# cipherflow-fhe/lattisense

Hardware: AMD Instinct MI355X
Metric: ckks_hmult_relin_rescale_throughput (higher is better)
Workload: dtype u64

## Files before the change

### lattisense_amd/csrc/build_flags.h

```cpp
#pragma once

#if (defined(LSA_NTT_DIAG_NO_TWIDDLE_LOADS) || defined(LSA_NTT_DIAG_COPY_ONLY) || defined(LSA_NTT_DIAG_COMPUTE_ONLY) || defined(LSA_NTT_DIAG_TW8) || \
     defined(LSA_KS_DIAG_NO_MATH) || defined(LSA_KS_DIAG_NO_STORE) || defined(LSA_BC_DIAG_NO_MATH) || defined(LSA_BC_DIAG_NO_STORE)) && \
    !defined(LSA_DIAG_BUILD)
#error "wrong-result diagnostic switches need -DLSA_DIAG_BUILD (use lattisense_amd.build --variant: it adds the flag and renames the library)"
#endif

#define LSA_BF_STR2(x) #x
#define LSA_BF_STR(x) LSA_BF_STR2(x)

#define LSA_BUILD_FLAGS_TEXT_1 ""
#ifdef LSA_DIAG_BUILD
#define LSA_BF_DIAG " LSA_DIAG_BUILD"
#else
#define LSA_BF_DIAG ""
#endif
#ifdef LSA_NTT_DIAG_NO_TWIDDLE_LOADS
#define LSA_BF_A " LSA_NTT_DIAG_NO_TWIDDLE_LOADS"
#else
#define LSA_BF_A ""
#endif
#ifdef LSA_NTT_DIAG_COPY_ONLY
#define LSA_BF_B " LSA_NTT_DIAG_COPY_ONLY"
#else
// ... 54 lines not shown
#else
#define LSA_BF_M ""
#endif
#ifdef LSA_BC_CARRY_COMPARES
#define LSA_BF_N " LSA_BC_CARRY_COMPARES"
#else
#define LSA_BF_N ""
#endif
#if defined(LSA_NTT_THREADS) && LSA_NTT_THREADS != 256
#define LSA_BF_O " LSA_NTT_THREADS=" LSA_BF_STR(LSA_NTT_THREADS)
#else
#define LSA_BF_O ""
#endif
#if defined(LSA_NTT_MAX_RHO) && LSA_NTT_MAX_RHO != 4
#define LSA_BF_P " LSA_NTT_MAX_RHO=" LSA_BF_STR(LSA_NTT_MAX_RHO)
#else
#define LSA_BF_P ""
#endif
#if defined(LSA_NTT_WAVES) && LSA_NTT_WAVES != 4
#define LSA_BF_Q " LSA_NTT_WAVES=" LSA_BF_STR(LSA_NTT_WAVES)
#else
#define LSA_BF_Q ""
#endif
#if defined(LSA_NTT_WAVES_FUSED) && LSA_NTT_WAVES_FUSED != 3
#define LSA_BF_R " LSA_NTT_WAVES_FUSED=" LSA_BF_STR(LSA_NTT_WAVES_FUSED)
#else
#define LSA_BF_R ""
#endif
#if defined(LSA_NTT_TAU) && LSA_NTT_TAU != 12
#define LSA_BF_S " LSA_NTT_TAU=" LSA_BF_STR(LSA_NTT_TAU)
#else
#define LSA_BF_S ""
#endif
#if defined(LSA_NTT_STORE_CHUNK) && LSA_NTT_STORE_CHUNK != 4
#define LSA_BF_T " LSA_NTT_STORE_CHUNK=" LSA_BF_STR(LSA_NTT_STORE_CHUNK)
#else
#define LSA_BF_T ""
#endif
#if defined(LSA_NTT_HEAD_ROUNDS) && LSA_NTT_HEAD_ROUNDS != 2
#define LSA_BF_U " LSA_NTT_HEAD_ROUNDS=" LSA_BF_STR(LSA_NTT_HEAD_ROUNDS)
#else
#define LSA_BF_U ""
#endif
#ifdef LSA_R16_BARRIERS
#define LSA_BF_X " LSA_R16_BARRIERS"
#else
#define LSA_BF_X ""
#endif
#if defined(LSA_R16_WAVES) && LSA_R16_WAVES != 4
#define LSA_BF_Y " LSA_R16_WAVES=" LSA_BF_STR(LSA_R16_WAVES)
#else
#define LSA_BF_Y ""
#endif
#ifdef LSA_NTT_NO_LAZY
#define LSA_BF_Z " LSA_NTT_NO_LAZY"
#else
#define LSA_BF_Z ""
#endif
#ifdef LSA_SHOUP_SINGLE_ASM
#define LSA_BF_AA " LSA_SHOUP_SINGLE_ASM"
#else
#define LSA_BF_AA ""
#endif
#ifdef LSA_AB_DPP_LO
#define LSA_BF_AB " LSA_AB_DPP_LO"
#else
#define LSA_BF_AB ""
#endif
#if defined(LSA_KSMAC_WAVES) && LSA_KSMAC_WAVES != 2
#define LSA_BF_AC " LSA_KSMAC_WAVES=" LSA_BF_STR(LSA_KSMAC_WAVES)
#else
#define LSA_BF_AC ""
#endif
#if defined(LSA_KSMAC_WAVES_FP) && LSA_KSMAC_WAVES_FP != 2
#define LSA_BF_AE " LSA_KSMAC_WAVES_FP=" LSA_BF_STR(LSA_KSMAC_WAVES_FP)
#else
#define LSA_BF_AE ""
#endif
#if defined(LSA_KSMAC_CHUNK) && LSA_KSMAC_CHUNK != 4
#define LSA_BF_AF " LSA_KSMAC_CHUNK=" LSA_BF_STR(LSA_KSMAC_CHUNK)
#else
#define LSA_BF_AF ""
#endif
#ifdef LSA_NTT_DIAG_TW8
#define LSA_BF_AD " LSA_NTT_DIAG_TW8"
#else
#define LSA_BF_AD ""
#endif
#ifdef LSA_LIFT_ROW_OUTER
#define LSA_BF_AG " LSA_LIFT_ROW_OUTER"
#else
#define LSA_BF_AG ""
#endif
#ifdef LSA_VARIANT_NAME
#define LSA_BF_V " variant=" LSA_BF_STR(LSA_VARIANT_NAME)
#else
#define LSA_BF_V ""
#endif
#ifdef LSA_AB_SWITCH
#define LSA_BF_W " LSA_AB_SWITCH=" LSA_BF_STR(LSA_AB_SWITCH)
#else
#define LSA_BF_W ""
#endif

#define LSA_BUILD_FLAGS_TEXT                                                                                              \
    LSA_BF_DIAG LSA_BF_A LSA_BF_B LSA_BF_C LSA_BF_D LSA_BF_E LSA_BF_F LSA_BF_G LSA_BF_H LSA_BF_I LSA_BF_J LSA_BF_K LSA_BF_L \
        LSA_BF_M LSA_BF_N LSA_BF_O LSA_BF_P LSA_BF_Q LSA_BF_R LSA_BF_S LSA_BF_T LSA_BF_U LSA_BF_V LSA_BF_W LSA_BF_X LSA_BF_Y LSA_BF_Z LSA_BF_AA LSA_BF_AB LSA_BF_AC LSA_BF_AD LSA_BF_AE LSA_BF_AF LSA_BF_AG
```

### lattisense_amd/csrc/kernels.hip

```cpp
#include <atomic>
#include <cstdlib>

#include "build_flags.h"
#include "lsa_internal.h"
#include "ntt_r16.h"
#include "plain_ops.h"
#include "poly_lincomb.h"
#include "tensor_sum.h"

namespace lsa {

const char* kernels_build_flags() { return LSA_BUILD_FLAGS_TEXT; }

static constexpr int TPB = 256;

#ifndef LSA_NTT_WAVES
#define LSA_NTT_WAVES 4
#endif

#if defined(LSA_NTT_DIAG_STAMPS)
#define LSA_STAMP(k)                                                                               \
    do {                                                                                           \
        if (a.diag && threadIdx.x == 0 && blockIdx.x < 8192) a.diag[blockIdx.x * 8 + (k)] = __builtin_amdgcn_s_memtime(); \
    } while (0)
// ... 136 lines not shown
}
static bool ntt_launch_r16(const NttPassArgs& a, int npass, bool fused, long long nblocks, hipStream_t s) {
    if (!sw::ntt_r16() || !ntt_r16_shape_ok(a, npass)) return false;
    const int fz = ntt_pass_fz(a, fused);
    void (*k)(NttPassArgs) = nullptr;
    if (a.lambda) {
        if (fz == 1 && a.fz_pro == 4 && sw::r16_pro()) k = a.mu == 8 ? &k_ntt_r16<0, 32, 8> : &k_ntt_r16<0, 32, 7>;
        else if (fz == 1 && a.fz_pro != 4 && a.mu == 8 && sw::r16_pro()) k = &k_ntt_r16<0, 1, 8>;
        else if (fz == 0) k = a.mu == 8 ? &k_ntt_r16<0, 0, 8> : &k_ntt_r16<0, 0, 7>;
    } else if (a.mu != 9 || sw::ntt_r8x3()) {
        switch (fz) {
            case 0: k = ntt_r16_second_pass<0>(a.mu); break;
            case 2: k = ntt_r16_second_pass<2>(a.mu); break;
            case 4: k = ntt_r16_second_pass<4>(a.mu); break;
            case 8: k = ntt_r16_second_pass<8>(a.mu); break;
            case 16: k = a.inverse ? ntt_r16_second_pass<16>(a.mu) : nullptr; break;
        }
    }
    if (!k) return false;
    hipLaunchKernelGGL(k, dim3((unsigned)nblocks), dim3(LSA_R16_THREADS), (size_t)LSA_R16_LDS_WORDS * sizeof(u64), s, a);
    LSA_HIP(hipGetLastError());
    return true;
}

#ifndef LSA_KSMAC_WAVES
#define LSA_KSMAC_WAVES 2
#endif
#ifndef LSA_KSMAC_WAVES_FP
#define LSA_KSMAC_WAVES_FP LSA_KSMAC_WAVES
#endif
template <int MU, bool FP, bool TAIL = false>
__global__ __launch_bounds__(LSA_R16_THREADS, FP ? LSA_KSMAC_WAVES_FP : LSA_KSMAC_WAVES) void k_ntt_r16_ksmac(KsFusedArgs g) {
    static_assert(!TAIL || (FP && MU <= 8), "the tail runs on the FP64 engine's eight- and seven-stage passes");
    extern __shared__ __attribute__((aligned(16))) u64 lds[];
    const int tid = threadIdx.x;
    const int T = g.L + g.np;
    long long bid = blockIdx.x;
    long long b;
    if (g.xcd_deal) {
        const long long slot = bid >> 3;
        b = slot % g.batch;
        bid = (slot / g.batch) * 8 + (bid & 7);
    } else {
        b = bid % g.batch;
        bid /= g.batch;
    }
    const int tl = g.tl_list[bid % g.n_tl], tile = (int)(bid / g.n_tl);
    NttPassArgs a;
    a.logn = g.logn;
    a.s_lo = g.logn - MU;
    a.mu = MU;
    a.lambda = 0;
    a.tau = 12;
    a.inverse = 0;
    a.apply_scale = 0;
    a.final_reduce = 1;
    a.fp_raw_in = g.fp_raw_in;
    a.fp_raw_out = 0;
    a.mods = g.mods;
    a.tw = g.tw;
    a.twd = g.twd;
    a.scale = nullptr;
    a.scaled = nullptr;
    a.src = g.ext;
    a.fz_pro = a.fz_epi = 0;
    a.fz_first = 0;
    NttBlockCtx bc;
    bc.tile = tile;
    bc.mod = tl < g.L ? tl : g.nq + (tl - g.L);
    bc.fp = FP;
    bc.b = (int)b;
    bc.row = 0;
    bc.tw_l = nullptr;
    bc.base_dst = 0;
    const R16Limb L = r16_limb(a, bc);
    const int kj = tl < g.L ? tl : g.klvl + 1 + (tl - g.L);
    const int own_d = tl < g.L ? tl / g.np : -1;
    int k, i;
    r16_lane<1, MU>(tid, k, i);
    const unsigned G1 = r16_G1<1, MU>(bc, k), G2 = (G1 << 4) + ((unsigned)i << (MU <= 8 ? 8 - MU : 0));
    u64 acc0[16], acc1[16];
#pragma unroll
    for (int e = 0; e < 16; e++) acc0[e] = acc1[e] = 0;
    for (int d = 0; d < g.beta; d++) {
        const bool own = d == own_d;
        if (!own) {
            bc.base_src = b * g.sext + ((long long)(d * T + tl) << g.logn);
            bc.row = d * T + tl;
            u64 v[16];
            r16_load_direct<1, false, 0, MU>(a, bc, tid, v);
            if constexpr (MU == 9) {
                r8x3_group<0>(v, a, bc, L, G1, i);
                r8x3_put<0>(k, i, lds, v);
                r16_sync<1>();
                r8x3_get<1>(k, i, lds, v);
                r8x3_group<1>(v, a, bc, L, G1, i);
                r8x3_put<1>(k, i, lds, v);
                r16_sync<1>();
                r8x3_get<2>(k, i, lds, v);
                r8x3_group<2>(v, a, bc, L, G1, i);
                r8x3_put<2>(k, i, lds, v);
            } else {
                r16_group<1, 0, MU>(v, a, bc, L, G1);
                r16_lds_put<1, 0, MU>(tid, lds, v);
                r16_sync<1>();
                r16_lds_get<1, 1, MU>(tid, lds, v);
                r16_group<1, 1, MU>(v, a, bc, L, G2);
                r16_lds_put<1, 1, MU>(tid, lds, v);
            }
            r16_sync<1>();
        }
        r16_mac_digit<MU, FP>(g, a, bc, L, tid, d, kj, own, b, tl, lds, acc0, acc1);
        r16_sync<1>();
    }
    if constexpr (TAIL) {
        a.src = g.tconv;
        int tt = tid, ttl = tl;
        long long tb = b;
        asm volatile("" : "+v"(tt), "+s"(ttl), "+s"(tb));
        int tk, ti;
        r16_lane<1, MU>(tt, tk, ti);
        const unsigned T1 = r16_G1<1, MU>(bc, tk), T2 = (T1 << 4) + ((unsigned)ti << (8 - MU));
        const double kd = g.tkd[ttl], k2d = g.tkd[g.L - 1 + ttl];
#pragma unroll 1
        for (int h = 0; h < 2; h++) {
            bc.row = h * g.L + ttl;
            bc.base_src = tb * g.stconv + ((long long)bc.row << g.logn);
            u64 v[16];
            r16_load_direct<1, false, 0, MU>(a, bc, tt, v);
            r16_group<1, 0, MU>(v, a, bc, L, T1);
            r16_lds_put<1, 0, MU>(tt, lds, v);
            r16_sync<1>();
            r16_lds_get<1, 1, MU>(tt, lds, v);
            r16_group<1, 1, MU>(v, a, bc, L, T2);
            r16_lds_put<1, 1, MU>(tt, lds, v);
            r16_sync<1>();
            r16_mac_tail<MU>(g, a, bc, L, tt, tb, ttl, h, kd, k2d, lds, acc0);
            r16_sync<1>();
#pragma unroll
            for (int e = 0; e < 16; e++) acc0[e] = acc1[e];
        }
        return;
    }
    r16_mac_store<MU, FP>(g, a, bc, L, tid, b, tl, acc0, acc1);
}

bool ks_fused_enabled(const Context& c) {
    if (!sw::ks_fused() || c.plan.npass != 2 || !c.fp_raw) return false;
    const NttPassShape& p = c.plan.pass[1];
    return p.tau == 12 && p.lambda == 0 && (p.mu == 7 || p.mu == 8 || p.mu == 9) && p.s_lo == c.logn - p.mu;
}

int ks_fused_engines(const Context& c) {
    return c.fp64_ntt ? sw::ks_fused_engines() : 0;
}

bool ks_fused_limb(const Context& c, int L, int tl) { return (ks_fused_engines(c) >> (c.fp_engine(c.qp_mod(L, tl)) ? 1 : 0)) & 1; }

bool launch_ntt_ksmac(Context& c, int level, const u64* cx, long long scx, u64* ext, long long sext, const Key& key, u64* acc,
                      long long sacc, int batch, hipStream_t s, const TensorFold* fold, KsFusedLimbs limbs, const KsTailOperands* tail) {
    if (batch <= 0) return true;
    if (!ks_fused_enabled(c) || (c.fp64_ntt && !key.fp)) return false;
    LSA_REQUIRE(key.level >= level, "key-switch key exported at a lower level than the ciphertext");
    LSA_REQUIRE((limbs == KS_FUSED_Q_TAIL) == (tail != nullptr), "fused key MAC: the tail launch and its operands go together");
    if (tail && (level < 1 || ks_fused_engines(c) != 2 || c.plan.pass[1].mu > 8)) return false;
    KsFusedArgs g{};
    if (tail) {
        g.tconv = tail->conv;
        g.stconv = tail->sconv;
        g.tout = tail->out;
        g.stout = tail->sout;
        g.tkd = reinterpret_cast<const double*>(c.tail_fp_vec(level));
    }
    g.ext = ext;
    g.cx = cx;
    g.key = key.data;
    g.keyd = key.fp;
    g.acc = acc;
    g.sext = sext;
    g.scx = scx;
    g.sacc = sacc;
    g.mods = c.d_mods;
    g.tw = c.d_psi;
    g.twd = c.d_psi_d;
    g.logn = c.logn;
    g.L = level + 1;
    g.np = c.np;
    g.nq = c.nq;
    g.beta = (g.L + c.np - 1) / c.np;
    g.klvl = key.level;
    g.kcomp = key.level + 1 + c.np;
    g.batch = batch;
    g.allow_fp64 = c.fp64_ntt;
    g.fp_raw_in = c.fp_raw;
    if (fold) {
        g.fa = fold->a;
        g.fb = fold->b;
        g.sfa = fold->sa;
        g.sfb = fold->sb;
        g.pfa = fold->pa;
        g.pfb = fold->pb;
        g.pf = c.pfold_vec(level);
    }
    const int T = g.L + c.np, mu = c.plan.pass[1].mu;
    LSA_REQUIRE(T <= 64, "fused key MAC: too many target limbs");
    const size_t lds_bytes = (size_t)LSA_R16_LDS_WORDS * sizeof(u64);
    for (int eng = 0; eng < 2; eng++) {
        g.n_tl = 0;
        int transforms = 0, q_targets = 0;
        for (int tl = 0; tl < T; tl++) {
            if (!ks_fused_limb(c, g.L, tl) || (int)c.fp_engine(c.qp_mod(g.L, tl)) != eng) continue;
            if (limbs == KS_FUSED_P && tl < g.L) continue;
            if (limbs == KS_FUSED_Q_TAIL && tl >= level) continue;
            g.tl_list[g.n_tl++] = (unsigned char)tl;
            transforms += g.beta - (tl < g.L ? 1 : 0);
            q_targets += tl < g.L;
        }
        if (!g.n_tl) continue;
        const long long nblocks = (long long)batch * g.n_tl * (1 << (c.logn - 12));
        LSA_REQUIRE(nblocks < (1LL << 31), "ntt: grid too large");
        g.xcd_deal = sw::ksmac_xcd() && ((g.n_tl << (c.logn - 12)) % 8 == 0) ? 1 : 0;
        if (tail) transforms += 2 * g.n_tl;
        const double ntt_bytes = 16.0 * c.n * transforms * batch / 2;
        const double fold_bytes = fold ? 3.0 * 8 * c.n * q_targets * batch : 0.0;
        ProfScope ps(c, PROF_NTT, ntt_bytes + fold_bytes + 8.0 * c.n * g.n_tl * (batch * ((double)g.beta + (tail ? 0.0 : 2.0)) + 2.0 * g.beta), s,
                     ntt_bytes);
        const dim3 grid((unsigned)nblocks), block(LSA_R16_THREADS);
        if (tail) {
            LSA_REQUIRE(eng == 1 && (mu == 8 || mu == 7), "fused key MAC: the tail runs on the FP64 engine's eight- and seven-stage passes");
            if (mu == 8) hipLaunchKernelGGL((k_ntt_r16_ksmac<8, true, true>), grid, block, lds_bytes, s, g);
            else hipLaunchKernelGGL((k_ntt_r16_ksmac<7, true, true>), grid, block, lds_bytes, s, g);
        } else if (mu == 9 && eng) hipLaunchKernelGGL((k_ntt_r16_ksmac<9, true>), grid, block, lds_bytes, s, g);
        else if (mu == 9) hipLaunchKernelGGL((k_ntt_r16_ksmac<9, false>), grid, block, lds_bytes, s, g);
        else if (mu == 8 && eng) hipLaunchKernelGGL((k_ntt_r16_ksmac<8, true>), grid, block, lds_bytes, s, g);
        else if (mu == 8) hipLaunchKernelGGL((k_ntt_r16_ksmac<8, false>), grid, block, lds_bytes, s, g);
        else if (eng) hipLaunchKernelGGL((k_ntt_r16_ksmac<7, true>), grid, block, lds_bytes, s, g);
        else hipLaunchKernelGGL((k_ntt_r16_ksmac<7, false>), grid, block, lds_bytes, s, g);
    }
    LSA_HIP(hipGetLastError());
    return true;
}

template <int FZ, int NT>
static void ntt_launch_variant(const NttPassArgs& a, long long nblocks, size_t lds_bytes, hipStream_t s) {
    if (lds_bytes > 65536) {
        static std::atomic<unsigned long long> raised{0};
        int dev = 0;
        LSA_HIP(hipGetDevice(&dev));
        const unsigned long long bit = 1ull << (dev & 63);
        if (!(raised.load(std::memory_order_acquire) & bit)) {
            LSA_HIP(hipFuncSetAttribute(reinterpret_cast<const void*>(&k_ntt_pass<FZ, NT>), hipFuncAttributeMaxDynamicSharedMemorySize, 160 * 1024));
            raised.fetch_or(bit, std::memory_order_release);
        }
    }
    hipLaunchKernelGGL((k_ntt_pass<FZ, NT>), dim3((unsigned)nblocks), dim3(NT), lds_bytes, s, a);
    LSA_HIP(hipGetLastError());
}

template <int NT>
static void ntt_launch_pass(const NttPassArgs& a, bool fused, long long nblocks, size_t lds_bytes, hipStream_t s) {
    LSA_REQUIRE((1 << a.tau) <= 2 * LSA_NTT_STAGE_PAIRS * NT, "ntt: tile larger than the staging registers");
    switch (ntt_pass_fz(a, fused)) {
        case 0: ntt_launch_variant<0, NT>(a, nblocks, lds_bytes, s); break;
        case 1: ntt_launch_variant<1, NT>(a, nblocks, lds_bytes, s); break;
        case 2: ntt_launch_variant<2, NT>(a, nblocks, lds_bytes, s); break;
        case 3: ntt_launch_variant<3, NT>(a, nblocks, lds_bytes, s); break;
        case 4: ntt_launch_variant<4, NT>(a, nblocks, lds_bytes, s); break;
        case 8: ntt_launch_variant<8, NT>(a, nblocks, lds_bytes, s); break;
        default:
            if constexpr (NT == LSA_NTT_THREADS) ntt_launch_variant<16, NT>(a, nblocks, lds_bytes, s);
            else LSA_REQUIRE(false, "ntt: the product prologue needs a tile of at most 4096 points");
    }
}

void launch_ntt(Context& c, const u64* src, u64* dst, int batch, long long batch_stride, int rows, const RowMap& rm,
                bool inverse, hipStream_t s) {
    launch_ntt(c, src, dst, batch, batch_stride, batch_stride, rows, rm, inverse, s);
}

void launch_ntt(Context& c, const u64* src, u64* dst, int batch, long long src_stride, long long dst_stride, int rows,
                const RowMap& rm, bool inverse, hipStream_t s, const NttFusion* fz, int passes) {
    if (batch <= 0 || rows <= 0) return;
    LSA_REQUIRE(rm.period >= 1 && rm.period <= LSA_MAX_PERIOD, "ntt: bad row-map period");
    NttPassArgs a{};
    a.batch = batch;
    a.rows = rows;
    a.mods = c.d_mods;
    a.scale = c.d_scale;
    a.diag = c.ntt_diag;
    a.scaled = c.d_scale_d;
    a.allow_fp64 = c.fp64_ntt;
    if (fz) {
        LSA_REQUIRE(!inverse || (fz->pro == 3 && !fz->epi), "inverse transforms take the product prologue only");
        LSA_REQUIRE(fz->pro != 3 || (inverse && !fz->epi && fz->a && fz->b && fz->limbs >= 1 && (passes & 1)),
                    "product prologue: an inverse transform from its first pass, two operands, no epilogue");
        LSA_REQUIRE(fz->pro != 4 || (!inverse && !fz->epi && fz->last && fz->limbs >= 1 && (passes & 1)),
                    "lift prologue: a forward transform from its first pass, one source row per polynomial, no epilogue");
        a.fz_epi = fz->epi;
        a.fz_pro = fz->pro;
        a.fz_limbs = fz->limbs;
        a.fz_base_polys = fz->base_polys;
        a.fz_ql_mod = fz->ql_mod;
        a.fz_a = fz->a;
        a.fz_a_stride = fz->a_stride;
        a.fz_a_rpp = fz->a_rpp;
        a.fz_base = fz->base;
        a.fz_base_stride = fz->base_stride;
        a.fz_base_rpp = fz->base_rpp;
        a.fz_k = fz->k;
        a.fz_out = fz->out;
        a.fz_out_stride = fz->out_stride;
        a.fz_out_rpp = fz->out_rpp;
        a.fz_last = fz->last;
        a.fz_last_stride = fz->last_stride;
        a.fz_last_rpp = fz->last_rpp;
        a.fz_k2 = fz->k2;
        a.fz_scatter = fz->scatter;
        LSA_REQUIRE(fz->epi != 2 || fz->k2, "merged tail needs its second factor");
        LSA_REQUIRE(!fz->scatter || fz->epi, "a scattered store needs an epilogue");
        LSA_REQUIRE(fz->epi != 3 || (!fz->pro && !fz->scatter && fz->a && fz->out), "pt_mul epilogue: plaintext and output, nothing else");
// ... 2089 lines not shown
```

### lattisense_amd/csrc/ntt_core.h

```cpp
#pragma once
#include "modarith.h"

#ifndef LSA_NTT_THREADS
#define LSA_NTT_THREADS 256
#endif
#define LSA_MAX_PERIOD 192
#if defined(LSA_EMULATE)
#include <cstdio>
#include <cstdlib>
#define LSA_EMU_CHECK(c) do { if (!(c)) { std::fprintf(stderr, "ntt replay: range invariant violated: %s (%s:%d)\n", #c, __FILE__, __LINE__); std::abort(); } } while (0)
#else
#define LSA_EMU_CHECK(c) do { } while (0)
#endif
#define LSA_ROW_SKIP 0xFF
#define LSA_FP64_MAX_BITS 47
#ifndef LSA_NTT_MAX_RHO
#define LSA_NTT_MAX_RHO 4
#endif

struct NttPassArgs {
    const u64* src;
    u64* dst;
    long long src_stride;
    long long dst_stride;
// ... 832 lines not shown
#endif
                }
                continue;
            }
            const u64* tws = tw + 2 * (1LL << s);
            u64 w[E / 2], ws[E / 2];
#if defined(LSA_NTT_DIAG_TW8)
            if (!TWU) {
                double wd[E / 2];
                ntt_load_tw_fp(reinterpret_cast<const double*>(tw) + (1LL << s), s, j, G, wd);
#pragma unroll
                for (int k = 0; k < (1 << j); k++) {
                    w[k] = (u64)__builtin_bit_cast(long long, wd[k]);
                    ws[k] = (w[k] << 3) | 1;
                }
            } else
#endif
#pragma unroll
            for (int k = 0; k < (1 << j); k++) {
                if (TWU) {
                    w[k] = LSA_CONST_PTR(u64, tws)[2 * ntt_tw_u_int(s, j, k) + 2u * ntt_tw_v_int(j, G)];
                    ws[k] = LSA_CONST_PTR(u64, tws)[2 * ntt_tw_u_int(s, j, k) + 2u * ntt_tw_v_int(j, G) + 1];
                } else {
                    ntt_load_pair(tws + 2 * ntt_tw_u_int(s, j, k) + 2u * ntt_tw_v_int(j, G), w[k], ws[k]);
                }
            }
#pragma unroll
            for (int e = 0; e < E; e++) {
                if ((e & half) == 0) {
                    const int k = e >> (RHO - j);
                    u64 U = v[e], V = v[e + half];
#if defined(LSA_NTT_DIAG_NO_TWIDDLE_LOADS)
                    const u64 wk = (u64)(G + 2 * k + 3), wsk = (u64)(G + 2 * k + 5) << 40;
#else
                    const u64 wk = w[k], wsk = ws[k];
#endif
#if defined(LSA_NTT_EXACT_BFLY)
                    v[e] = csub(U + V, q2);
                    v[e + half] = shoup_mul_lazy(sub64(U + q2, V), wk, wsk, q);
#else
                    LSA_EMU_CHECK(U < q4 && V < q4);
                    v[e] = csub_sign(U + V, nq4);
                    v[e + half] = shoup_mul_approx(sub64(U + q4, V), wk, wsk, nq);
                    LSA_EMU_CHECK(v[e] < q4 && v[e + half] < q4);
#endif
                }
            }
        }
    }
}

template <int RHO, bool TWU = false>
LSA_HD void ntt_group_int(u64 (&v)[1 << RHO], bool inverse, const u64* tw, int s_base, unsigned G, u64 q, bool scale_here, u64 sc0, u64 sc0s,
                          u64 sc1, u64 sc1s) {
    if (!inverse && ntt_int_lazy(q)) ntt_group_int_impl<RHO, TWU, true>(v, false, tw, s_base, G, q, false, 0, 0, 0, 0);
    else ntt_group_int_impl<RHO, TWU, false>(v, inverse, tw, s_base, G, q, scale_here, sc0, sc0s, sc1, sc1s);
}

template <int RHO, bool LIN, int NT, bool TWL = false>
LSA_HD void ntt_phase_sub(const NttPassArgs& a, const NttBlockCtx& bc, int tid, u64* lds, int sig0) {
    constexpr int E = 1 << RHO;
    const ModDev md = a.mods[bc.mod];
    const u64* tw = TWL ? bc.tw_l : a.tw + (((long long)bc.mod << a.logn) << 1);
    const int beta0 = a.lambda + a.mu - sig0 - RHO;
    const int ngroups = 1 << (a.tau - RHO);
    const bool scale_here = a.inverse && a.apply_scale && a.s_lo + sig0 == 0;
    const u64* sc = a.scale + 4 * bc.mod;
    const u64 sc0 = scale_here ? sc[0] : 0, sc0s = scale_here ? sc[1] : 0, sc1 = scale_here ? sc[2] : 0, sc1s = scale_here ? sc[3] : 0;
    for (int gid = tid; gid < ngroups; gid += NT) {
        int lbase = ((gid >> beta0) << (beta0 + RHO)) | (gid & ((1 << beta0) - 1));
        const int ad0 = lds_addr(lbase), adst = !LIN ? 0 : beta0 ? (1 << beta0) + (1 << (beta0 - 4)) : 1;
        u64 v[E];
#pragma unroll
        for (int e = 0; e < E; e++) v[e] = lds[LIN ? ad0 + e * adst : lds_addr(lbase + (e << beta0))];
        int r = (lbase >> a.lambda) & ((1 << a.mu) - 1);
        int H = ntt_hi_index(a, bc.tile, lbase);
        int G = (H << sig0) + (r >> (a.mu - sig0));
        ntt_group_int<RHO>(v, a.inverse != 0, tw, a.s_lo + sig0, (unsigned)G, md.q, scale_here, sc0, sc0s, sc1, sc1s);
#pragma unroll
        for (int e = 0; e < E; e++) lds[LIN ? ad0 + e * adst : lds_addr(lbase + (e << beta0))] = v[e];
    }
}

template <int RHO, bool TWU = false>
LSA_HD void ntt_group_fp(double (&v)[1 << RHO], bool inverse, const double* tw , int s_base, unsigned G, double q, double qinv,
                         bool scale_here, double sc0, double sc1, bool long_pass) {
    constexpr int E = 1 << RHO;
    if (!inverse) {
#pragma unroll
        for (int j = 0; j < RHO; j++) {
            const int half = E >> (j + 1);
            const int s = s_base + j;
            double w[E / 2];
            if (TWU) {
#pragma unroll
                for (int k = 0; k < (1 << j); k++) w[k] = LSA_CONST_PTR(double, tw + (1LL << s))[ntt_tw_pos_fp(s, j, G, k)];
            } else {
                ntt_load_tw_fp(tw + (1LL << s), s, j, G, w);
            }
#pragma unroll
            for (int e = 0; e < E; e++) {
                if ((e & half) == 0) {
#if defined(LSA_NTT_DIAG_NO_TWIDDLE_LOADS)
                    const double T = fp_modmul(v[e + half], (double)(G + j + 3), q, qinv);
#else
                    const double T = fp_modmul(v[e + half], w[e >> (RHO - j)], q, qinv);
#endif
                    const double U = v[e];
                    LSA_EMU_CHECK(__builtin_fabs(U) < 2251799813685248.0 && __builtin_fabs(v[e + half]) < 2251799813685248.0);
                    v[e] = U + T;
                    v[e + half] = U - T;
                }
            }
        }
        if (long_pass) {
#pragma unroll
            for (int e = 0; e < E; e++) v[e] = fp_reduce(v[e], q, qinv);
        }
    } else {
#pragma unroll
        for (int j = RHO - 1; j >= 0; j--) {
            const int half = E >> (j + 1);
            const int s = s_base + j;
            if (j == 0 && scale_here) {
#pragma unroll
                for (int e = 0; e < half; e++) {
                    const double U = v[e], V = v[e + half];
                    v[e] = fp_modmul(U + V, sc0, q, qinv);
                    v[e + half] = fp_modmul(U - V, sc1, q, qinv);
                }
                continue;
            }
            double w[E / 2];
            if (TWU) {
#pragma unroll
                for (int k = 0; k < (1 << j); k++) w[k] = LSA_CONST_PTR(double, tw + (1LL << s))[ntt_tw_pos_fp(s, j, G, k)];
            } else {
                ntt_load_tw_fp(tw + (1LL << s), s, j, G, w);
            }
#pragma unroll
            for (int e = 0; e < E; e++) {
                if ((e & half) == 0) {
                    const double U = v[e], V = v[e + half];
                    v[e] = U + V;
                    v[e + half] = fp_modmul(U - V, w[e >> (RHO - j)], q, qinv);
                }
            }
        }
#pragma unroll
        for (int e = 0; e < E; e++) v[e] = fp_reduce(v[e], q, qinv);
    }
}

template <int RHO, bool LIN, int NT, bool TWL = false>
LSA_HD void ntt_phase_sub_fp(const NttPassArgs& a, const NttBlockCtx& bc, int tid, u64* lds, int sig0) {
    constexpr int E = 1 << RHO;
    const double q = (double)a.mods[bc.mod].q, qinv = 1.0 / q;
    const double* tw = TWL ? reinterpret_cast<const double*>(bc.tw_l) : a.twd + ((long long)bc.mod << a.logn);
    const int beta0 = a.lambda + a.mu - sig0 - RHO;
    const int ngroups = 1 << (a.tau - RHO);
    const bool scale_here = a.inverse && a.apply_scale && a.s_lo + sig0 == 0;
    const double sc0 = scale_here ? a.scaled[2 * bc.mod] : 0.0, sc1 = scale_here ? a.scaled[2 * bc.mod + 1] : 0.0;
    for (int gid = tid; gid < ngroups; gid += NT) {
        int lbase = ((gid >> beta0) << (beta0 + RHO)) | (gid & ((1 << beta0) - 1));
        const int ad0 = lds_addr(lbase), adst = !LIN ? 0 : beta0 ? (1 << beta0) + (1 << (beta0 - 4)) : 1;
        double v[E];
#pragma unroll
        for (int e = 0; e < E; e++) v[e] = d_from_bits(lds[LIN ? ad0 + e * adst : lds_addr(lbase + (e << beta0))]);
        int r = (lbase >> a.lambda) & ((1 << a.mu) - 1);
        int H = ntt_hi_index(a, bc.tile, lbase);
        int G = (H << sig0) + (r >> (a.mu - sig0));
        ntt_group_fp<RHO>(v, a.inverse != 0, tw, a.s_lo + sig0, (unsigned)G, q, qinv, scale_here, sc0, sc1, a.mu > 9);
#pragma unroll
        for (int e = 0; e < E; e++) lds[LIN ? ad0 + e * adst : lds_addr(lbase + (e << beta0))] = d_to_bits(v[e]);
    }
}

LSA_HD int ntt_split(int mu, int* rho ) {
    const int n = (mu + LSA_NTT_MAX_RHO - 1) / LSA_NTT_MAX_RHO;
    if ((mu > 12 || mu == 10) && LSA_NTT_MAX_RHO == 4) {
        for (int i = 0; i < n; i++) rho[i] = 4;
        rho[n - 2] = mu - 4 * (n - 1);
        return n;
    }
    const int base = mu / n, extra = mu % n;
    for (int i = 0; i < n; i++) rho[i] = base + (i < extra ? 1 : 0);
    return n;
}

template <bool LIN, int NT, bool TWL = false>
LSA_HD void ntt_phase_sub_sel(const NttPassArgs& a, const NttBlockCtx& bc, int tid, u64* lds, int sig0, int rho) {
    if (bc.fp) {
        switch (rho) {
            case 1: ntt_phase_sub_fp<1, LIN, NT, TWL>(a, bc, tid, lds, sig0); break;
            case 2: ntt_phase_sub_fp<2, LIN, NT, TWL>(a, bc, tid, lds, sig0); break;
#if LSA_NTT_MAX_RHO >= 4
            case 3: ntt_phase_sub_fp<3, LIN, NT, TWL>(a, bc, tid, lds, sig0); break;
            default: ntt_phase_sub_fp<4, LIN, NT, TWL>(a, bc, tid, lds, sig0); break;
#elif LSA_NTT_MAX_RHO == 3
            default: ntt_phase_sub_fp<3, LIN, NT, TWL>(a, bc, tid, lds, sig0); break;
#else
            default: break;
#endif
        }
        return;
    }
    switch (rho) {
        case 1: ntt_phase_sub<1, LIN, NT, TWL>(a, bc, tid, lds, sig0); break;
        case 2: ntt_phase_sub<2, LIN, NT, TWL>(a, bc, tid, lds, sig0); break;
#if LSA_NTT_MAX_RHO >= 4
        case 3: ntt_phase_sub<3, LIN, NT, TWL>(a, bc, tid, lds, sig0); break;
        default: ntt_phase_sub<4, LIN, NT, TWL>(a, bc, tid, lds, sig0); break;
#elif LSA_NTT_MAX_RHO == 3
        default: ntt_phase_sub<3, LIN, NT, TWL>(a, bc, tid, lds, sig0); break;
#else
        default: break;
#endif
// ... 12 lines not shown
```

### lattisense_amd/csrc/ntt_r16.h

```cpp
#pragma once
#include "ntt_core.h"

#define LSA_R16_THREADS 256
#define LSA_R16_LDS_WORDS (272 * 16)

LSA_HD bool ntt_r16_shape_ok(const NttPassArgs& a, int npass) {
    if (npass != 2 || a.tau != 12) return false;
    if (a.mu == 9) return a.s_lo == a.logn - 9 && a.lambda == 0;
    if (a.mu != 8 && a.mu != 7) return false;
    return (a.s_lo == 0 && a.lambda == 12 - a.mu) || (a.s_lo == a.logn - a.mu && a.lambda == 0);
}

template <int PASS, int MU>
LSA_HD int r16_lds(int k, int i) {
    const int p = i + (i >> 4);
    return PASS == 0 ? (p << (12 - MU)) + k : k * ((1 << MU) + (1 << (MU - 4))) + p;
}
template <int PASS, int MU>
LSA_HD long long r16_x(const NttPassArgs& a, int tile, int k, int i) {
    return PASS == 0 ? ((long long)tile << (12 - MU)) + ((long long)i << (a.logn - MU)) + k : ((long long)tile << 12) + (k << MU) + i;
}
template <int MU, int IMAGE>
LSA_HD int r16_pt(int i, int e) {
    return IMAGE == 0 ? i + (e << (MU - 4)) : 16 * i + e;
// ... 471 lines not shown
        } else {
            u64 w[8];
#pragma unroll
            for (int e = 0; e < 8; e++) w[e] = v[r8x3_slot<IMAGE>(g, e)];
            ntt_group_int<3, false>(w, a.inverse != 0, L.tw, s_base, G, L.md.q, false, 0, 0, 0, 0);
#pragma unroll
            for (int e = 0; e < 8; e++) v[r8x3_slot<IMAGE>(g, e)] = w[e];
        }
    }
}
template <int IMAGE>
LSA_HD void r8x3_put(int k, int i, u64* lds, const u64 (&v)[16]) {
#pragma unroll
    for (int E = 0; E < 16; E++) lds[r16_lds<1, 9>(k, r8x3_pt<IMAGE>(i, E))] = v[E];
}
template <int IMAGE>
LSA_HD void r8x3_get(int k, int i, const u64* lds, u64 (&v)[16]) {
#pragma unroll
    for (int E = 0; E < 16; E++) v[E] = lds[r16_lds<1, 9>(k, r8x3_pt<IMAGE>(i, E))];
}
template <int FZ>
LSA_HD void r8x3_phase(const NttPassArgs& a, const NttBlockCtx& bc, int tid, u64* lds, int phase, u64 (&v)[16]) {
    const R16Limb L = r16_limb(a, bc);
    const int k = tid >> 5, i = tid & 31;
    const unsigned G1 = r16_G1<1, 9>(bc, k);
    if (!a.inverse) {
        if (phase == 0) {
            r16_load_direct<1, false, 0, 9>(a, bc, tid, v);
            r8x3_group<0>(v, a, bc, L, G1, i);
            r8x3_put<0>(k, i, lds, v);
        } else if (phase == 1) {
            r8x3_get<1>(k, i, lds, v);
            r8x3_group<1>(v, a, bc, L, G1, i);
            r8x3_put<1>(k, i, lds, v);
        } else if (phase == 2) {
            r8x3_get<2>(k, i, lds, v);
            r8x3_group<2>(v, a, bc, L, G1, i);
            r8x3_put<2>(k, i, lds, v);
        } else {
            r16_store_coalesced<(FZ & 2) != 0, 9, (FZ & 4) != 0, (FZ & 8) != 0>(a, bc, tid, lds);
        }
    } else {
        if (phase == 0) {
            r16_load_coalesced<false, 9, (FZ & 16) != 0>(a, bc, tid, lds);
        } else if (phase == 1) {
            r8x3_get<2>(k, i, lds, v);
            r8x3_group<2>(v, a, bc, L, G1, i);
            r8x3_put<2>(k, i, lds, v);
        } else if (phase == 2) {
            r8x3_get<1>(k, i, lds, v);
            r8x3_group<1>(v, a, bc, L, G1, i);
            r8x3_put<1>(k, i, lds, v);
        } else {
            r8x3_get<0>(k, i, lds, v);
            r8x3_group<0>(v, a, bc, L, G1, i);
            r16_store_direct<1, false, 0, 9>(a, bc, tid, v);
        }
    }
}

struct KsFusedArgs {
    const u64* ext;
    const u64* cx;
    const u64* key;
    const double* keyd;
    u64* acc;
    long long sext, scx, sacc;
    const ModDev* mods;
    const u64* tw;
    const double* twd;
    int logn, L, np, nq, beta, kcomp, klvl, batch, allow_fp64, fp_raw_in;
    int xcd_deal;
    int n_tl;
    unsigned char tl_list[64];
    const u64* fa;
    const u64* fb;
    long long sfa, sfb, pfa, pfb;
    const u64* pf;
    const u64* tconv;
    u64* tout;
    long long stconv, stout;
    const double* tkd;
};

template <int MU, bool FP>
LSA_HD void r16_mac_digit(const KsFusedArgs& g, const NttPassArgs& a, const NttBlockCtx& bc, const R16Limb& L, int tid, int d, int kj,
                          bool own, long long b, int tl, const u64* lds, u64 (&acc0)[16], u64 (&acc1)[16]) {
    const long long N = 1LL << g.logn;
    const u64* k0 = g.key + ((long long)(2 * d) * g.kcomp + kj) * N;
    const u64* k1 = k0 + (long long)g.kcomp * N;
    const double* k0d = g.keyd + ((long long)(2 * d) * g.kcomp + kj) * N;
    const double* k1d = k0d + (long long)g.kcomp * N;
    const u64* own_src = g.cx + b * g.scx + (long long)tl * N;
    const u64 q = L.md.q, qinv = L.md.qinv;
    const bool lazy = ntt_int_lazy(q);
    const u64 one_s = L.tw[1];
#ifndef LSA_KSMAC_CHUNK
#define LSA_KSMAC_CHUNK 4
#endif
    constexpr int CH = LSA_KSMAC_CHUNK;
    if (own && g.fa) {
        const u64* pa0 = g.fa + b * g.sfa + (long long)tl * N;
        const u64* pb0 = g.fb + b * g.sfb + (long long)tl * N;
        const u64 pm = g.pf[tl];
        const double pd = (double)g.pf[g.L + tl];
#pragma unroll 1
        for (int m = 0; m < 8; m++) {
            int k, i;
            r16_pair_pos<MU>(tid, m, k, i);
            const long long x = r16_x<1, MU>(a, bc.tile, k, i);
            u64 va0[2], va1[2], vb0[2], vb1[2], ka[2], kb[2];
            ntt_load_data_pair(pa0 + x, va0[0], va0[1]);
            ntt_load_data_pair(pa0 + g.pfa + x, va1[0], va1[1]);
            ntt_load_data_pair(pb0 + x, vb0[0], vb0[1]);
            ntt_load_data_pair(pb0 + g.pfb + x, vb1[0], vb1[1]);
            if (FP) {
                ntt_load_pair(reinterpret_cast<const u64*>(k0d + x), ka[0], ka[1]);
                ntt_load_pair(reinterpret_cast<const u64*>(k1d + x), kb[0], kb[1]);
            } else {
                ntt_load_pair(k0 + x, ka[0], ka[1]);
                ntt_load_pair(k1 + x, kb[0], kb[1]);
            }
#pragma unroll
            for (int j = 0; j < 2; j++) {
                const int e = 2 * m + j;
                if (FP) {
                    const double a0 = u52_to_double(va0[j]), a1 = u52_to_double(va1[j]);
                    const double b0 = u52_to_double(vb0[j]), b1 = u52_to_double(vb1[j]);
                    const double d2 = fp_modmul(a1, b1, L.q, L.qinv);
                    const double p0 = fp_modmul(b0, pd, L.q, L.qinv), p1 = fp_modmul(b1, pd, L.q, L.qinv);
                    acc0[e] = d_to_bits(d_from_bits(acc0[e]) + fp_modmul(d2, d_from_bits(ka[j]), L.q, L.qinv) +
                                        fp_modmul(p0, a0, L.q, L.qinv));
                    acc1[e] = d_to_bits(d_from_bits(acc1[e]) + fp_modmul(d2, d_from_bits(kb[j]), L.q, L.qinv) +
                                        fp_modmul(p1, a0, L.q, L.qinv) + fp_modmul(p0, a1, L.q, L.qinv));
                } else {
                    const u64 d2 = mont_mul_lazy(va1[j], mont_mul_lazy(vb1[j], L.md.r2, q, qinv), q, qinv);
                    const u64 p0 = mont_mul_lazy(vb0[j], pm, q, qinv), p1 = mont_mul_lazy(vb1[j], pm, q, qinv);
                    u64 s0 = csub_sign(acc0[e] + mont_mul_lazy(d2, ka[j], q, qinv), 0 - 2 * q);
                    u64 s1 = csub_sign(acc1[e] + mont_mul_lazy(d2, kb[j], q, qinv), 0 - 2 * q);
                    s1 = csub_sign(s1 + mont_mul_lazy(va0[j], p1, q, qinv), 0 - 2 * q);
                    acc0[e] = csub_sign(s0 + mont_mul_lazy(va0[j], p0, q, qinv), 0 - 2 * q);
                    acc1[e] = csub_sign(s1 + mont_mul_lazy(va1[j], p0, q, qinv), 0 - 2 * q);
                }
            }
        }
        return;
    }
#pragma unroll
    for (int m0 = 0; m0 < 8; m0 += CH) {
        u64 v[2 * CH], ka[2 * CH], kb[2 * CH];
        long long xs[CH];
#pragma unroll
        for (int m = 0; m < CH; m++) {
            int k, i;
            r16_pair_pos<MU>(tid, m0 + m, k, i);
            xs[m] = r16_x<1, MU>(a, bc.tile, k, i);
            if (own) {
                ntt_load_data_pair(own_src + xs[m], v[2 * m], v[2 * m + 1]);
            } else {
                v[2 * m] = lds[r16_lds<1, MU>(k, i)];
                v[2 * m + 1] = lds[r16_lds<1, MU>(k, i + 1)];
            }
            if (FP) {
                ntt_load_pair(reinterpret_cast<const u64*>(k0d + xs[m]), ka[2 * m], ka[2 * m + 1]);
                ntt_load_pair(reinterpret_cast<const u64*>(k1d + xs[m]), kb[2 * m], kb[2 * m + 1]);
            } else {
// ... 78 lines not shown
```

Before: 15800.

## Cache FP64 NTT twiddles in LDS across digits in fused key-switch MAC kernel

In the fused key-switch MAC kernel's FP64 path for the 8- and 7-stage passes, each block now loads its twiddle factors into extra LDS once before the digit loop. Every digit's forward NTT and the tail transform then read them from LDS instead of reloading them from global memory. The kernel's dynamic shared memory grows past 64 KB, so a one-time per-device attribute raise is added before launch. The larger LDS footprint may reduce occupancy.

```diff
diff --git a/lattisense_amd/csrc/build_flags.h b/lattisense_amd/csrc/build_flags.h
--- a/lattisense_amd/csrc/build_flags.h
+++ b/lattisense_amd/csrc/build_flags.h
@@ -160,6 +160,11 @@
 #else
 #define LSA_BF_AF ""
 #endif
+#if defined(LSA_KSMAC_TWCACHE) && LSA_KSMAC_TWCACHE != 1
+#define LSA_BF_AH " LSA_KSMAC_TWCACHE=" LSA_BF_STR(LSA_KSMAC_TWCACHE)
+#else
+#define LSA_BF_AH ""
+#endif
 #ifdef LSA_NTT_DIAG_TW8
 #define LSA_BF_AD " LSA_NTT_DIAG_TW8"
 #else
@@ -183,4 +188,4 @@
 
 #define LSA_BUILD_FLAGS_TEXT                                                                                              \
     LSA_BF_DIAG LSA_BF_A LSA_BF_B LSA_BF_C LSA_BF_D LSA_BF_E LSA_BF_F LSA_BF_G LSA_BF_H LSA_BF_I LSA_BF_J LSA_BF_K LSA_BF_L \
-        LSA_BF_M LSA_BF_N LSA_BF_O LSA_BF_P LSA_BF_Q LSA_BF_R LSA_BF_S LSA_BF_T LSA_BF_U LSA_BF_V LSA_BF_W LSA_BF_X LSA_BF_Y LSA_BF_Z LSA_BF_AA LSA_BF_AB LSA_BF_AC LSA_BF_AD LSA_BF_AE LSA_BF_AF LSA_BF_AG
+        LSA_BF_M LSA_BF_N LSA_BF_O LSA_BF_P LSA_BF_Q LSA_BF_R LSA_BF_S LSA_BF_T LSA_BF_U LSA_BF_V LSA_BF_W LSA_BF_X LSA_BF_Y LSA_BF_Z LSA_BF_AA LSA_BF_AB LSA_BF_AC LSA_BF_AD LSA_BF_AE LSA_BF_AF LSA_BF_AG LSA_BF_AH
diff --git a/lattisense_amd/csrc/kernels.hip b/lattisense_amd/csrc/kernels.hip
--- a/lattisense_amd/csrc/kernels.hip
+++ b/lattisense_amd/csrc/kernels.hip
@@ -242,6 +242,12 @@
     u64 acc0[16], acc1[16];
 #pragma unroll
     for (int e = 0; e < 16; e++) acc0[e] = acc1[e] = 0;
+    constexpr bool TWC = ks_fused_twc(MU, FP);
+    double* const twc = reinterpret_cast<double*>(lds + LSA_R16_LDS_WORDS);
+    if constexpr (TWC) {
+        r16_twc_fill<MU>(twc, tid, L, G1, G2);
+        r16_sync<1>();
+    }
     for (int d = 0; d < g.beta; d++) {
         const bool own = d == own_d;
         if (!own) {
@@ -260,6 +266,16 @@
                 r8x3_get<2>(k, i, lds, v);
                 r8x3_group<2>(v, a, bc, L, G1, i);
                 r8x3_put<2>(k, i, lds, v);
+            } else if constexpr (TWC) {
+                double w[15];
+                r16_twc_get<MU, 0>(twc, tid, w);
+                r16_group_twc<0, MU>(v, false, L, w);
+                r16_lds_put<1, 0, MU>(tid, lds, v);
+                r16_sync<1>();
+                r16_twc_get<MU, 1>(twc, tid, w);
+                r16_lds_get<1, 1, MU>(tid, lds, v);
+                r16_group_twc<1, MU>(v, false, L, w);
+                r16_lds_put<1, 1, MU>(tid, lds, v);
             } else {
                 r16_group<1, 0, MU>(v, a, bc, L, G1);
                 r16_lds_put<1, 0, MU>(tid, lds, v);
@@ -288,12 +304,24 @@
             bc.base_src = tb * g.stconv + ((long long)bc.row << g.logn);
             u64 v[16];
             r16_load_direct<1, false, 0, MU>(a, bc, tt, v);
-            r16_group<1, 0, MU>(v, a, bc, L, T1);
-            r16_lds_put<1, 0, MU>(tt, lds, v);
-            r16_sync<1>();
-            r16_lds_get<1, 1, MU>(tt, lds, v);
-            r16_group<1, 1, MU>(v, a, bc, L, T2);
-            r16_lds_put<1, 1, MU>(tt, lds, v);
+            if constexpr (TWC) {
+                double w[15];
+                r16_twc_get<MU, 0>(twc, tt, w);
+                r16_group_twc<0, MU>(v, false, L, w);
+                r16_lds_put<1, 0, MU>(tt, lds, v);
+                r16_sync<1>();
+                r16_twc_get<MU, 1>(twc, tt, w);
+                r16_lds_get<1, 1, MU>(tt, lds, v);
+                r16_group_twc<1, MU>(v, false, L, w);
+                r16_lds_put<1, 1, MU>(tt, lds, v);
+            } else {
+                r16_group<1, 0, MU>(v, a, bc, L, T1);
+                r16_lds_put<1, 0, MU>(tt, lds, v);
+                r16_sync<1>();
+                r16_lds_get<1, 1, MU>(tt, lds, v);
+                r16_group<1, 1, MU>(v, a, bc, L, T2);
+                r16_lds_put<1, 1, MU>(tt, lds, v);
+            }
             r16_sync<1>();
             r16_mac_tail<MU>(g, a, bc, L, tt, tb, ttl, h, kd, k2d, lds, acc0);
             r16_sync<1>();
@@ -303,6 +331,22 @@
         return;
     }
     r16_mac_store<MU, FP>(g, a, bc, L, tid, b, tl, acc0, acc1);
+}
+
+template <int MU, bool FP, bool TAIL = false>
+static void ks_fused_launch(dim3 grid, dim3 block, hipStream_t s, const KsFusedArgs& g) {
+    constexpr size_t lds_bytes = ks_fused_lds_bytes(MU, FP);
+    if (lds_bytes > 65536) {
+        static std::atomic<unsigned long long> raised{0};
+        int dev = 0;
+        LSA_HIP(hipGetDevice(&dev));
+        const unsigned long long bit = 1ull << (dev & 63);
+        if (!(raised.load(std::memory_order_acquire) & bit)) {
+            LSA_HIP(hipFuncSetAttribute(reinterpret_cast<const void*>(&k_ntt_r16_ksmac<MU, FP, TAIL>), hipFuncAttributeMaxDynamicSharedMemorySize, (int)lds_bytes));
+            raised.fetch_or(bit, std::memory_order_release);
+        }
+    }
+    hipLaunchKernelGGL((k_ntt_r16_ksmac<MU, FP, TAIL>), grid, block, lds_bytes, s, g);
 }
 
 bool ks_fused_enabled(const Context& c) {
@@ -364,7 +408,6 @@
     }
     const int T = g.L + c.np, mu = c.plan.pass[1].mu;
     LSA_REQUIRE(T <= 64, "fused key MAC: too many target limbs");
-    const size_t lds_bytes = (size_t)LSA_R16_LDS_WORDS * sizeof(u64);
     for (int eng = 0; eng < 2; eng++) {
         g.n_tl = 0;
         int transforms = 0, q_targets = 0;
@@ -388,14 +431,14 @@
         const dim3 grid((unsigned)nblocks), block(LSA_R16_THREADS);
         if (tail) {
             LSA_REQUIRE(eng == 1 && (mu == 8 || mu == 7), "fused key MAC: the tail runs on the FP64 engine's eight- and seven-stage passes");
-            if (mu == 8) hipLaunchKernelGGL((k_ntt_r16_ksmac<8, true, true>), grid, block, lds_bytes, s, g);
-            else hipLaunchKernelGGL((k_ntt_r16_ksmac<7, true, true>), grid, block, lds_bytes, s, g);
-        } else if (mu == 9 && eng) hipLaunchKernelGGL((k_ntt_r16_ksmac<9, true>), grid, block, lds_bytes, s, g);
-        else if (mu == 9) hipLaunchKernelGGL((k_ntt_r16_ksmac<9, false>), grid, block, lds_bytes, s, g);
-        else if (mu == 8 && eng) hipLaunchKernelGGL((k_ntt_r16_ksmac<8, true>), grid, block, lds_bytes, s, g);
-        else if (mu == 8) hipLaunchKernelGGL((k_ntt_r16_ksmac<8, false>), grid, block, lds_bytes, s, g);
-        else if (eng) hipLaunchKernelGGL((k_ntt_r16_ksmac<7, true>), grid, block, lds_bytes, s, g);
-        else hipLaunchKernelGGL((k_ntt_r16_ksmac<7, false>), grid, block, lds_bytes, s, g);
+            if (mu == 8) ks_fused_launch<8, true, true>(grid, block, s, g);
+            else ks_fused_launch<7, true, true>(grid, block, s, g);
+        } else if (mu == 9 && eng) ks_fused_launch<9, true>(grid, block, s, g);
+        else if (mu == 9) ks_fused_launch<9, false>(grid, block, s, g);
+        else if (mu == 8 && eng) ks_fused_launch<8, true>(grid, block, s, g);
+        else if (mu == 8) ks_fused_launch<8, false>(grid, block, s, g);
+        else if (eng) ks_fused_launch<7, true>(grid, block, s, g);
+        else ks_fused_launch<7, false>(grid, block, s, g);
     }
     LSA_HIP(hipGetLastError());
     return true;
diff --git a/lattisense_amd/csrc/ntt_core.h b/lattisense_amd/csrc/ntt_core.h
--- a/lattisense_amd/csrc/ntt_core.h
+++ b/lattisense_amd/csrc/ntt_core.h
@@ -938,9 +938,9 @@
     }
 }
 
-template <int RHO, bool TWU = false>
+template <int RHO, bool TWU = false, bool TWC = false>
 LSA_HD void ntt_group_fp(double (&v)[1 << RHO], bool inverse, const double* tw , int s_base, unsigned G, double q, double qinv,
-                         bool scale_here, double sc0, double sc1, bool long_pass) {
+                         bool scale_here, double sc0, double sc1, bool long_pass, const double* twc = nullptr) {
     constexpr int E = 1 << RHO;
     if (!inverse) {
 #pragma unroll
@@ -948,7 +948,10 @@
             const int half = E >> (j + 1);
             const int s = s_base + j;
             double w[E / 2];
-            if (TWU) {
+            if (TWC) {
+#pragma unroll
+                for (int k = 0; k < (1 << j); k++) w[k] = twc[(1 << j) - 1 + k];
+            } else if (TWU) {
 #pragma unroll
                 for (int k = 0; k < (1 << j); k++) w[k] = LSA_CONST_PTR(double, tw + (1LL << s))[ntt_tw_pos_fp(s, j, G, k)];
             } else {
@@ -988,7 +991,10 @@
                 continue;
             }
             double w[E / 2];
-            if (TWU) {
+            if (TWC) {
+#pragma unroll
+                for (int k = 0; k < (1 << j); k++) w[k] = twc[(1 << j) - 1 + k];
+            } else if (TWU) {
 #pragma unroll
                 for (int k = 0; k < (1 << j); k++) w[k] = LSA_CONST_PTR(double, tw + (1LL << s))[ntt_tw_pos_fp(s, j, G, k)];
             } else {
diff --git a/lattisense_amd/csrc/ntt_r16.h b/lattisense_amd/csrc/ntt_r16.h
--- a/lattisense_amd/csrc/ntt_r16.h
+++ b/lattisense_amd/csrc/ntt_r16.h
@@ -577,6 +577,97 @@
     long long stconv, stout;
     const double* tkd;
 };
+
+#ifndef LSA_KSMAC_TWCACHE
+#define LSA_KSMAC_TWCACHE 1
+#endif
+template <int MU>
+struct R16Twc {
+    static_assert(MU == 8 || MU == 7, "the cached-twiddle loop covers the radix-16 x radix-2^(MU-4) passes");
+    static constexpr int R2 = MU - 4, NG = 16 >> R2, E2 = (1 << R2) - 1;
+    static constexpr int PG = (E2 - 1) / 2;
+    static constexpr int SHARED = 16 << (12 - MU);
+    static constexpr int WAVE = 64 * NG + 128 * NG * PG;
+    static constexpr int WORDS = SHARED + (LSA_R16_THREADS / 64) * WAVE;
+    static LSA_HD int shared(int k, int e) { return 16 * k + 1 + e; }
+    static LSA_HD int priv(int tid, int g, int e) {
+        const int base = SHARED + (tid >> 6) * WAVE, lane = tid & 63;
+        return e == 0 ? base + 64 * g + lane : base + 64 * NG + 128 * (g * PG + ((e - 1) >> 1)) + 2 * lane + ((e - 1) & 1);
+    }
+};
+constexpr bool ks_fused_twc(int mu, bool fp) { return LSA_KSMAC_TWCACHE != 0 && fp && (mu == 8 || mu == 7); }
+static_assert(R16Twc<8>::WORDS == R16Twc<7>::WORDS, "one cache size for both splits");
+constexpr size_t ks_fused_lds_bytes(int mu, bool fp) {
+    return (size_t)(LSA_R16_LDS_WORDS + (ks_fused_twc(mu, fp) ? R16Twc<8>::WORDS : 0)) * sizeof(u64);
+}
+LSA_HD void r16_twc_ld2(const double* p, double& x, double& y) {
+#if defined(__HIP_DEVICE_COMPILE__)
+    const double2 v = *reinterpret_cast<const double2*>(p);
+    x = v.x;
+    y = v.y;
+#else
+    x = p[0];
+    y = p[1];
+#endif
+}
+template <int MU>
+LSA_HD void r16_twc_fill(double* twc, int tid, const R16Limb& L, unsigned G1, unsigned G2) {
+    typedef R16Twc<MU> C;
+    int k, i;
+    r16_lane<1, MU>(tid, k, i);
+    if (i == 0) {
+#pragma unroll
+        for (int j = 0; j < 4; j++) {
+            double w[8];
+            const int s = L.s_lo + j;
+            ntt_load_tw_fp(L.twd + (1LL << s), s, j, G1, w);
+#pragma unroll
+            for (int kk = 0; kk < (1 << j); kk++) twc[C::shared(k, (1 << j) - 1 + kk)] = w[kk];
+        }
+    }
+#pragma unroll
+    for (int g = 0; g < C::NG; g++) {
+#pragma unroll
+        for (int j = 0; j < C::R2; j++) {
+            double w[8];
+            const int s = L.s_lo + 4 + j;
+            ntt_load_tw_fp(L.twd + (1LL << s), s, j, G2 + (unsigned)g, w);
+#pragma unroll
+            for (int kk = 0; kk < (1 << j); kk++) twc[C::priv(tid, g, (1 << j) - 1 + kk)] = w[kk];
+        }
+    }
+}
+template <int MU, int HI>
+LSA_HD void r16_twc_get(const double* twc, int tid, double (&w)[15]) {
+    typedef R16Twc<MU> C;
+    if (HI == 0) {
+        int k, i;
+        r16_lane<1, MU>(tid, k, i);
+        w[0] = twc[C::shared(k, 0)];
+#pragma unroll
+        for (int e = 1; e < 15; e += 2) r16_twc_ld2(twc + C::shared(k, e), w[e], w[e + 1]);
+        return;
+    }
+#pragma unroll
+    for (int g = 0; g < C::NG; g++) {
+        w[g * C::E2] = twc[C::priv(tid, g, 0)];
+#pragma unroll
+        for (int e = 1; e < C::E2; e += 2) r16_twc_ld2(twc + C::priv(tid, g, e), w[g * C::E2 + e], w[g * C::E2 + e + 1]);
+    }
+}
+template <int HI, int MU>
+LSA_HD void r16_group_twc(u64 (&v)[16], bool inverse, const R16Limb& L, const double (&w)[15]) {
+    constexpr int R = HI ? MU - 4 : 4, NG = 16 >> R, E = 1 << R;
+#pragma unroll
+    for (int g = 0; g < NG; g++) {
+        double d[E];
+#pragma unroll
+        for (int e = 0; e < E; e++) d[e] = d_from_bits(v[g * E + e]);
+        ntt_group_fp<R, false, true>(d, inverse, nullptr, 0, 0u, L.q, L.qinv, false, 0.0, 0.0, false, w + g * (E - 1));
+#pragma unroll
+        for (int e = 0; e < E; e++) v[g * E + e] = d_to_bits(d[e]);
+    }
+}
 
 template <int MU, bool FP>
 LSA_HD void r16_mac_digit(const KsFusedArgs& g, const NttPassArgs& a, const NttBlockCtx& bc, const R16Limb& L, int tid, int d, int kj,
```

After: 16010 (median of 6 runs). +1.3%, better.
